# SynthAIr/T-VQ-VAE-TrajGen

Measured on AMD Instinct MI355X. Metric: stage1+stage2 train steps/sec on synthetic (B,C,T) trajectories, 1/2/4/8 GPU, higher is better.
Workload: dtype fp32; 1 GPU; stage1 VQ-VAE + stage2 MaskGIT joint train step, per-GPU batch (B=256,C=6,T=256), K=512, configs/config.yaml architecture; global_batch=256, seq_len=256, parallelism=dp1, launch=hipgraph

## Files before the change

include/tvq.h:

```cpp
#ifndef TVQ_H
#define TVQ_H
#include <stdint.h>

#ifdef __cplusplus
extern "C" {
#endif

#define TVQ_OK 0
#define TVQ_ERR_ARG -1
#define TVQ_ERR_LAUNCH -2

typedef void* tvq_stream_t;

const char* tvq_last_error(void);
int tvq_abi_version(void);
const char* tvq_source_hash(void);
const char* tvq_build_extra(void);
int tvq_counter_pool(int64_t device, int32_t* zeroed, int64_t n);
int tvq_counter_capture(int64_t begin);
int tvq_fill(float* p, int64_t n, float value, tvq_stream_t stream);
int tvq_fill_i64(int64_t* p, int64_t n, int64_t value, tvq_stream_t stream);
int tvq_fill2(float* p, float a, float* q, float b, tvq_stream_t stream);
int tvq_add_i64(int64_t* p, int64_t value, tvq_stream_t stream);
int tvq_sum4(const float* a, const float* b, const float* c, const float* d, float* out,
// ... 307 lines not shown
int tvq_upsample_nearest_bwd(const float* dy, int64_t R, int64_t Lin, int64_t Lout, float* dx,
                             tvq_stream_t stream);
int tvq_gelu_fwd(const float* x, int64_t n, float* y, tvq_stream_t stream);
int tvq_ffn_fwd(const float* xn, const float* r, int64_t M, int64_t D, const float* W1,
                const float* b1, const float* W2, const float* b2, const float* gate, float p,
                const int64_t* seed_ptr, uint64_t offset, float* y, float* pre, float* hd,
                tvq_stream_t stream);
int tvq_ffn_bwd(const float* gy, const float* pre, int64_t M, int64_t D, const float* W1,
                const float* W2, const float* gate, float p, const int64_t* seed_ptr,
                uint64_t offset, float* d_pre, float* dxn, float* gy_gated, tvq_stream_t stream);
int tvq_gelu_bwd(const float* dy, const float* x, int64_t n, float* dx, tvq_stream_t stream);
int64_t tvq_attn_branch_workspace(int64_t B, int64_t D);
int tvq_attn_branch_fwd(const float* x, int64_t B, int64_t S, int64_t D, int64_t heads,
                        const float* g, float nscale, const float* Wqkv, const float* Wo,
                        const float* gate, float drop_p, const int64_t* seed_ptr, uint64_t offset,
                        float* y, float* xn, float* inv, float* qkv, float* o, float* lse,
                        tvq_stream_t stream);
int tvq_attn_branch_bwd(const float* gy, const float* x, int64_t B, int64_t S, int64_t D,
                        int64_t heads, const float* g, float nscale, const float* inv,
                        const float* Wqkv, const float* Wo, const float* gate, float drop_p,
                        const int64_t* seed_ptr, uint64_t offset, const float* qkv, const float* o,
                        const float* lse, float* dx, float* dqkv, float* gy_gated, float* dg,
                        int64_t accumulate, float* workspace, tvq_stream_t stream);


int64_t tvq_prior_lf_eval_workspace(int64_t depth, int64_t K, int64_t n, int64_t n_classes);
int tvq_prior_lf_eval(const int64_t* s, int64_t B, int64_t n, int64_t s_stride,
                      const int64_t* cls_idx, int64_t n_classes, int64_t width,
                      const float* const* weights, int64_t depth, int64_t K, float ln_eps,
                      float* logits, void* workspace, tvq_stream_t stream);
int tvq_prior_lf_eval_sample(const int64_t* s, int64_t B, int64_t n, int64_t s_stride,
                             const int64_t* cls_idx, int64_t n_classes, int64_t width,
                             const float* const* weights, int64_t depth, int64_t K, float ln_eps,
                             int64_t mask_id, const float* gumbel, const int64_t* seed_ptr,
                             uint64_t offset, int64_t* sampled, float* selp, float* logits,
                             void* workspace, int64_t workspace_ready, tvq_stream_t stream);
int tvq_prior_lf_eval_sample_cfg(const int64_t* s, int64_t B, int64_t n, int64_t s_stride,
                                 const int64_t* cls_idx, int64_t n_classes, int64_t width,
                                 const float* const* weights, int64_t depth, int64_t K,
                                 float ln_eps, float cfg_scale, int64_t mask_id,
                                 const float* gumbel, const int64_t* seed_ptr, uint64_t offset,
                                 int64_t* sampled, float* selp, float* logits, void* workspace,
                                 int64_t workspace_ready, tvq_stream_t stream);

int tvq_maskgit_sample(const float* logits, int64_t sb, int64_t sn, int64_t B, int64_t n,
                       int64_t K, const int64_t* s_in, int64_t mask_id, const float* gumbel,
// ... 126 lines not shown
```

t-vq-vae-trajgen_amd/timevqvae/hip/_native.py:

```python
import ctypes
import os
import threading

import torch

_HERE = os.path.dirname(os.path.abspath(__file__))
LIB_PATH = os.environ.get(
    "TVQ_HIP_LIB", os.path.join(os.path.dirname(os.path.dirname(_HERE)), "lib", "libtvq_hip.so"))

P = ctypes.c_void_p
I64 = ctypes.c_int64
I32 = ctypes.c_int
F32 = ctypes.c_float

SIGNATURES = {}
_lib = None
_lock = threading.Lock()


def sig(name, *argtypes, restype=I32):
    SIGNATURES[name] = (list(argtypes), restype)


CSRC = os.path.join(os.path.dirname(os.path.dirname(_HERE)), "csrc")
# ... 142 lines not shown
sig("tvq_attention_fwd", P, I64, P, I64, P, I64, P, I64, P, I64, I64, I64, I64, F32, F32, P, U64, P)
sig("tvq_attention_bwd", P, I64, P, I64, P, I64, P, I64, P, I64, P, I64, I64, I64, I64, F32, F32, P,
    U64, P, P, P, I64, P)
sig("tvq_embedding_fwd", P, I64, I64, P, P, I64, I64, F32, P, U64, P)
sig("tvq_embedding_bwd_workspace", I64, I64, restype=I64)
sig("tvq_embedding_bwd", P, I64, I64, P, I64, I64, P, I64, I64, F32, P, U64, P, P)
sig("tvq_masked_ce_workspace", I64, restype=I64)
sig("tvq_drop_first_token", P, I64, I64, I64, P, I64, P)
sig("tvq_masked_ce_fwd", P, I64, I64, I64, P, P, P, P, P, P)
sig("tvq_masked_ce_bwd", P, I64, I64, I64, P, P, P, P, P, P, I64, P)
sig("tvq_mask_tokens", P, I64, I64, I64, P, U64, P, P, P, P, P)
sig("tvq_upsample_nearest", P, I64, I64, I64, P, P)
sig("tvq_upsample_nearest_bwd", P, I64, I64, I64, P, P)
sig("tvq_gelu_fwd", P, I64, P, P)
sig("tvq_gelu_bwd", P, P, I64, P, P)
sig("tvq_prior_lf_eval_workspace", I64, I64, I64, I64, restype=I64)
sig("tvq_prior_lf_eval", P, I64, I64, I64, P, I64, I64, P, I64, I64, F32, P, P, P)
sig("tvq_ffn_fwd", P, P, I64, I64, P, P, P, P, P, F32, P, U64, P, P, P, P)
sig("tvq_ffn_bwd", P, P, I64, I64, P, P, P, F32, P, U64, P, P, P, P)
sig("tvq_attn_branch_workspace", I64, I64, restype=I64)
sig("tvq_attn_branch_fwd", P, I64, I64, I64, I64, P, F32, P, P, P, F32, P, U64, P, P, P, P, P, P, P)
sig("tvq_attn_branch_bwd", P, P, I64, I64, I64, I64, P, F32, P, P, P, P, F32, P, U64, P, P, P, P, P,
    P, P, I64, P, P)
sig("tvq_prior_lf_eval_sample", P, I64, I64, I64, P, I64, I64, P, I64, I64, F32, I64, P, P, U64,
    P, P, P, P, I64, P)
sig("tvq_prior_lf_eval_sample_cfg", P, I64, I64, I64, P, I64, I64, P, I64, I64, F32, F32, I64, P, P,
    U64, P, P, P, P, I64, P)
sig("tvq_maskgit_sample", P, I64, I64, I64, I64, I64, P, I64, P, P, U64, P, P, P)
sig("tvq_tied_logits_sample_workspace", I64, I64, I64, restype=I64)
sig("tvq_tied_logits_sample", P, I64, I64, P, I64, P, I64, I64, P, I64, P, P, U64, P, P, P, P, P)
sig("tvq_tied_logits_sample_cfg", P, P, I64, I64, P, I64, P, I64, I64, F32, P, I64, P, P, U64, P, P,
    P, P, P)
sig("tvq_maskgit_remask", P, I64, I64, I64, F32, P, P, U64, P, I64, P, P, P)
sig("tvq_conv_packcache_begin", I64, P, I64, P)
sig("tvq_conv_packcache_end")
sig("tvq_conv_packcache_release", I64)
sig("tvq_conv_packcache_pause", I64)
sig("tvq_conv_packcache_entries", restype=I64)
sig("tvq_conv_wgrad_defer_begin")
sig("tvq_conv_wgrad_defer_flush", P)
sig("tvq_wgrad_defer_begin_stream", P)
sig("tvq_conv_wgrad_defer_pause", I64)
sig("tvq_rocket_apply", P, I64, I64, I64, P, P, P, P, P, P, I64, P, P)
sig("tvq_fe_conv1d_out_len", I64, I64, I64, I64, I64, restype=I64)
sig("tvq_fe_ws_weight", P, I64, I64, F32, P, P)
sig("tvq_fe_conv1d", P, I64, I64, I64, P, P, I64, I64, I64, I64, I64, I64, P, P, I64, P)
# ... 123 lines not shown
```

t-vq-vae-trajgen_amd/timevqvae/hip/xf.py:

```python
import contextlib
import math
import os

import torch

from . import rng, streams, wgrad
from ._native import call, grad_sink, ptr, stream_ptr, value
from .conv import _keep
from .linear import _bias_grad_rows, gemm, weight_grad


def _rows(x):
    D = x.shape[-1]
    return x.reshape(-1, D), x.numel() // D, D


class _RMSNorm(torch.autograd.Function):
    @staticmethod
    def forward(ctx, x, g, scale):
        x2, M, D = _rows(x.contiguous())
        y = torch.empty_like(x2)
        inv = torch.empty(M, device=x.device, dtype=torch.float32)
        call("tvq_rmsnorm_fwd", ptr(x2), M, D, ptr(g), float(scale), ptr(y), ptr(inv), stream_ptr())
        ctx.save_for_backward(x2, g, inv)
# ... 272 lines not shown
                        gemm(dqkv, 1, L, xn, D, 1, L, D, M, out=sink, ldc=D, accumulate=True)
            else:
                dW = gemm(dqkv, 1, L, xn, D, 1, L, D, M)
                dws = [dW[i * D:(i + 1) * D] for i in range(3)]
        dwo = weight_grad(gg if gg is not None else g2, o, wo, M, D, D, ctx.wg_tag) if need[5] else None
        return (dx.reshape(B, S, D), None if sink_g is not None else dg, *dws, dwo, None, None, None,
                None)


def attn_branch_supported(x, g, attn):
    if not (FUSED_ATTN and x.is_cuda and x.dim() == 3 and x.shape[-1] == 128 and x.shape[1] <= 32
            and attn.heads == 2):
        return False
    ws = (g, attn.to_q.weight, attn.to_k.weight, attn.to_v.weight, attn.to_out.weight)
    return all(w.dtype == torch.float32 and w.is_cuda and w.is_contiguous() and
               w.data_ptr() % 16 == 0 for w in ws) and tuple(attn.to_q.weight.shape) == (128, 128)


def attn_branch(x, g, attn, gate, p):
    return _AttnBranch.apply(x, g, attn.to_q.weight, attn.to_k.weight, attn.to_v.weight,
                             attn.to_out.weight, gate, int(attn.heads), float(p), int(attn._site))


class _Attention(torch.autograd.Function):
    @staticmethod
    def forward(ctx, q, k, v, heads, drop_p, site):
        B, S, HD = q.shape
        Dh = HD // heads
        q, k, v = q.contiguous(), k.contiguous(), v.contiguous()
        o = torch.empty_like(q)
        lse = torch.empty(B * heads * S, device=q.device)
        seed = rng.seed_tensor(q.device) if drop_p > 0 else None
        off = rng.call_offset(site) if drop_p > 0 else 0
        scale = Dh ** -0.5
        call("tvq_attention_fwd", ptr(q), HD, ptr(k), HD, ptr(v), HD, ptr(o), HD, ptr(lse), B,
             heads, S, Dh, float(scale), float(drop_p), ptr(seed), off, stream_ptr())
        ctx.save_for_backward(q, k, v, o, lse)
        ctx.cfg = (heads, drop_p, off, scale)
        ctx.seed = seed
        return o

    @staticmethod
    def backward(ctx, go):
        q, k, v, o, lse = ctx.saved_tensors
        heads, drop_p, off, scale = ctx.cfg
        B, S, HD = q.shape
# ... 395 lines not shown
```

t-vq-vae-trajgen_amd/timevqvae/models/bidirectional_transformer.py:

```python
import os
import random
from typing import Union

import torch
import torch.nn as nn

from ..hip import rng, streams
from ..hip.conv import PackCache, bn_eval_fusable, conv2d, conv2d_bn_eval
from ..hip.linear import gemm, linear, weight_product
from ..hip.norm import bn_snake
from ..hip.xf import (attn_branch, attn_branch_supported, batch_colsum, drop_first_token,
                      embed_assemble, embedding, fused_ff, fused_ff_supported, gelu,
                      layer_norm, linear_act, masked_cross_entropy, prior_lf_eval,
                      prior_lf_eval_sample,
                      prior_lf_eval_supported, prior_lf_eval_workspace, qkv_attention, rmsnorm, rmsnorm_res,
                      upsample_nearest_t)
from ..hip._native import call, grad_sink, ptr, stream_ptr, value
from ..hip.sample import (codebook_gather_nchw, full_tokens, maskgit_sample, tied_logits_sample,
                          tied_logits_sample_cfg)
from ..hip.upscale import supported as ups_supported
from ..hip.upscale import (hf_embed_folded, hf_embed_supported, upsample_conv_gelu,
                           upsample_conv_gelu_bn_eval)

FUSED_SAMPLE = True
UPS_ON_TOKENS = True
HEAD_FOLD = True
HF_EMBED_FOLD = True


class RMSNorm(nn.Module):
    def __init__(self, dim):
        super().__init__()
        self.scale = dim ** 0.5
        self.g = nn.Parameter(torch.ones(dim))

    def forward(self, x):
        return rmsnorm(x, self.g)
# ... 74 lines not shown
        self.register_buffer("_touched", torch.ones(n), persistent=False)
        for i, layer in enumerate(self.layers):
            for p in layer.parameters():
                p._tvq_gate = (self, i)
        self._site = rng.new_site()
        self._epoch = -1
        self._touched_host = [1.0] * n

    def _draw_branches(self, device):
        from ..hip.optim import grad_epoch
        fresh = self._epoch != grad_epoch()
        self._epoch = grad_epoch()
        n = len(self.layers)
        if rng.decisions_on_device():
            call("tvq_layer_drop", ptr(rng.seed_tensor(device)), rng.call_offset(self._site),
                 float(self.layer_dropout), n, ptr(self._keep), ptr(self._touched),
                 int(not fresh), stream_ptr())
            return None
        keep = [0.0 if random.random() < self.layer_dropout else 1.0 for _ in range(n)]
        self._touched_host = keep if fresh else [max(a, b) for a, b in zip(self._touched_host, keep)]
        self._touched.copy_(torch.tensor(self._touched_host))
        return keep

    def forward(self, x):
        keep = None
        device_gates = False
        if self.training and self.layer_dropout > 0.0:
            keep = self._draw_branches(x.device)
            device_gates = keep is None
        elif self.training and self._touched_host != [1.0] * len(self.layers):
            self._touched_host = [1.0] * len(self.layers)
            self._touched.fill_(1.0)
        for i, (norms, block, _) in enumerate(self.layers):
            if keep is not None and keep[i] == 0.0:
                continue
            gate = self._keep[i:i + 1] if device_gates else None
            if isinstance(norms[0], RMSNorm):
                if isinstance(block, Attention) and attn_branch_supported(x, norms[0].g, block):
                    x = attn_branch(x, norms[0].g, block, gate,
                                    block.dropout if self.training else 0.0)
                    continue
                n, r = rmsnorm_res(x, norms[0].g)
                x = block(n, residual=r, gate=gate)
            else:
                x = block(norms[0](x), residual=x, gate=gate)
        return self.final_norm(x)


class ContinuousTransformerWrapper(nn.Module):
    def __init__(self, dim_in, dim_out, max_seq_len, attn_layers, use_abs_pos_emb=False,
                 post_emb_norm=True):
        super().__init__()
        if use_abs_pos_emb:
            raise NotImplementedError("abs pos emb is off on the path (use_abs_pos_emb=False)")
        dim = attn_layers.dim
        self.max_seq_len = max_seq_len
        self.post_emb_norm = LayerNorm(dim) if post_emb_norm else nn.Identity()
        self.attn_layers = attn_layers
        self.project_in = nn.Linear(dim_in, dim, bias=False)
        self.project_out = nn.Linear(dim, dim_out, bias=False)

    def forward(self, x):
        return self.forward_projected(linear(x, self.project_in.weight))

    def forward_projected(self, x, project_out=True):
        x = self.post_emb_norm(x)
        if not project_out:
            return self.attn_layers(x)
        x = self.attn_layers(x)
        return linear(x, self.project_out.weight)


class _Dropout(torch.autograd.Function):
    @staticmethod
    def forward(ctx, x, p, site):
        x = x.contiguous()
        y = torch.empty_like(x)
        seed = rng.seed_tensor(x.device)
        off = rng.call_offset(site)
        call("tvq_dropout_bwd", ptr(x), x.numel(), float(p), ptr(seed), off, ptr(y), stream_ptr())
        ctx.cfg = (p, off)
        ctx.seed = seed
        return y

    @staticmethod
    def backward(ctx, g):
        p, off = ctx.cfg
        g = g.contiguous()
        dx = torch.empty_like(g)
        call("tvq_dropout_bwd", ptr(g), g.numel(), float(p), ptr(ctx.seed), off, ptr(dx), stream_ptr())
        return dx, None, None

# ... 374 lines not shown
```

Baseline: 260.6 steps/s.

## Fuse D=32 transformer layer (LN, attention, FFN, norms) into one HIP kernel

Adds a whole-layer fused forward and backward kernel for the D=32, single-head, S<=128 transformer blocks. One workgroup per batch element computes the optional post-embedding LayerNorm, RMSNorm, QKV projection, softmax attention with dropout, output projection, residual, the FFN with GELU and dropout, and the optional final norm. Weights stay in registers and K/V in LDS, using MFMA 32x32x2 f32. This removes many small kernel launches and round trips of activations through global memory. The cost is a large, shape-specialised kernel with extra saved tensors, while the weight gradients still go through separate GEMMs.

New measurement: 261.3 steps/s, median of 6. No clear change (+0.3%).

```diff
diff --git a/include/tvq.h b/include/tvq.h
--- a/include/tvq.h
+++ b/include/tvq.h
@@ -353,6 +353,15 @@
                         const int64_t* seed_ptr, uint64_t offset, const float* qkv, const float* o,
                         const float* lse, float* dx, float* dqkv, float* gy_gated, float* dg,
                         int64_t accumulate, float* workspace, tvq_stream_t stream);
+int64_t tvq_xlayer32_workspace(int64_t B);
+int tvq_xlayer32_fwd(const float* x, int64_t B, int64_t S, int64_t D, int64_t heads,
+                     const void* const* params, float p_attn, float p_ff, const int64_t* seed_ptr,
+                     uint64_t off_attn, uint64_t off_ff, void* const* bufs, tvq_stream_t stream);
+int tvq_xlayer32_bwd(const float* gy, const float* x, int64_t B, int64_t S, int64_t D,
+                     int64_t heads, const void* const* params, float p_attn, float p_ff,
+                     const int64_t* seed_ptr, uint64_t off_attn, uint64_t off_ff,
+                     const void* const* saved, void* const* outs, void* const* dgains,
+                     int64_t accumulate_mask, float* workspace, tvq_stream_t stream);
 
 
 int64_t tvq_prior_lf_eval_workspace(int64_t depth, int64_t K, int64_t n, int64_t n_classes);
diff --git a/t-vq-vae-trajgen_amd/csrc/tvq_xlayer32.hip b/t-vq-vae-trajgen_amd/csrc/tvq_xlayer32.hip
--- /dev/null
+++ b/t-vq-vae-trajgen_amd/csrc/tvq_xlayer32.hip
@@ -0,0 +1,709 @@
+#include <math.h>
+
+#include "tvq_common.h"
+#include "tvq_conv_internal.h"
+#include "tvq_ff.h"
+#include "tvq_reduce.h"
+
+namespace tvq {
+
+namespace x32 {
+
+constexpr int D = 32, DH = 64, T = 256, SMAX = 128, LP = 65;
+constexpr int MAT = SMAX * LP;
+constexpr float LN_EPS = 1e-5f;
+
+struct Args {
+  const float *ln_gamma, *g1, *Wq, *Wk, *Wv, *Wo, *gate_a, *g2, *W1, *b1, *W2, *b2, *gate_f, *g3;
+  const float *x, *gy;
+  float *xl, *xn1, *qkv, *o, *lse, *x1, *xn2, *pre, *hd, *x2, *y;
+  float *dx, *dqkv, *gyg_a, *d_pre, *gyg_f, *slab;
+  const int64_t* seed_ptr;
+  uint64_t off_a, off_f;
+  float nscale, scale, p_a, ds_a, p_f, ds_f;
+  int B, S;
+};
+
+__device__ __forceinline__ int wid() { return __builtin_amdgcn_readfirstlane(threadIdx.x >> 6); }
+
+__device__ __forceinline__ bool keep(uint64_t seed, int64_t bh, int S, int i, int j, float p) {
+  return uniform01(seed, ((uint64_t)bh * S + i) * S + j) >= p;
+}
+template <bool KEYS>
+__device__ __forceinline__ uint32_t keep_bits(uint64_t seed, int64_t bh, int S, int q, int k0, int h,
+                                              float p) {
+  uint32_t m = 0;
+#pragma unroll
+  for (int r = 0; r < 16; ++r) {
+    const int o = k0 + ff_crow(r, h);
+    m |= (uint32_t)(KEYS ? keep(seed, bh, S, q, o, p) : keep(seed, bh, S, o, q, p)) << r;
+  }
+  return m;
+}
+__device__ __forceinline__ float gelu(float x) {
+  return 0.5f * x * (1.0f + erff(x * 0.70710678118654752440f));
+}
+__device__ __forceinline__ float gelu_grad(float x) {
+  const float cdf = 0.5f * (1.0f + erff(x * 0.70710678118654752440f));
+  const float pdf = 0.39894228040143267794f * expf(-0.5f * x * x);
+  return cdf + x * pdf;
+}
+
+__device__ __forceinline__ floatx16 load_fm(const float* __restrict__ p, int h) {
+  floatx16 t;
+#pragma unroll
+  for (int g = 0; g < 4; ++g) {
+    const float4 v = *reinterpret_cast<const float4*>(p + 8 * g + 4 * h);
+    t[4 * g] = v.x; t[4 * g + 1] = v.y; t[4 * g + 2] = v.z; t[4 * g + 3] = v.w;
+  }
+  return t;
+}
+__device__ __forceinline__ void store_fm(float* __restrict__ p, int h, const floatx16& t) {
+#pragma unroll
+  for (int g = 0; g < 4; ++g)
+    *reinterpret_cast<float4*>(p + 8 * g + 4 * h) =
+        make_float4(t[4 * g], t[4 * g + 1], t[4 * g + 2], t[4 * g + 3]);
+}
+__device__ __forceinline__ floatx16 wload(const float* __restrict__ W, int ld, int r0, int k0, int lane) {
+  return load_fm(W + (int64_t)(r0 + (lane & 31)) * ld + k0, lane >> 5);
+}
+__device__ __forceinline__ floatx16 wload_t(const float* __restrict__ W, int ld, int k0, int c0, int lane) {
+  floatx16 a;
+  const float* wc = W + c0 + (lane & 31);
+#pragma unroll
+  for (int t = 0; t < 16; ++t) a[t] = wc[(int64_t)(k0 + ff_crow(t, lane >> 5)) * ld];
+  return a;
+}
+__device__ __forceinline__ floatx16 mma16(const floatx16& a, const floatx16& b, floatx16 acc) {
+#pragma unroll
+  for (int t = 0; t < 16; ++t) acc = __builtin_amdgcn_mfma_f32_32x32x2f32(a[t], b[t], acc, 0, 0, 0);
+  return acc;
+}
+__device__ __forceinline__ floatx16 mma_rows(const float* __restrict__ M, int r0, int c0, int lane,
+                                             const floatx16& b, floatx16 acc) {
+  const float* m = M + (r0 + (lane & 31)) * LP + c0 + 4 * (lane >> 5);
+#pragma unroll
+  for (int t = 0; t < 16; ++t)
+    acc = __builtin_amdgcn_mfma_f32_32x32x2f32(m[(t & 3) + 8 * (t >> 2)], b[t], acc, 0, 0, 0);
+  return acc;
+}
+__device__ __forceinline__ bool live(int S, int r0, int g) { return r0 + 8 * g < S; }
+__device__ __forceinline__ floatx16 mma_cols(const float* __restrict__ M, int r0, int c0, int lane,
+                                             const floatx16& b, floatx16 acc, int S) {
+  const float* m = M + (r0 + 4 * (lane >> 5)) * LP + c0 + (lane & 31);
+#pragma unroll
+  for (int g = 0; g < 4; ++g)
+    if (live(S, r0, g))
+#pragma unroll
+      for (int e = 0; e < 4; ++e)
+        acc = __builtin_amdgcn_mfma_f32_32x32x2f32(m[(e + 8 * g) * LP], b[4 * g + e], acc, 0, 0, 0);
+  return acc;
+}
+__device__ __forceinline__ void stage(float* __restrict__ M, int tok, int c0, int h, const floatx16& t) {
+#pragma unroll
+  for (int r = 0; r < 16; ++r) M[tok * LP + c0 + ff_crow(r, h)] = t[r];
+}
+__device__ __forceinline__ float half_sum(float v) { return v + __shfl_xor(v, 32, 64); }
+
+__device__ __forceinline__ float rms_inv(const floatx16& x) {
+  float ss = 0.f;
+#pragma unroll
+  for (int r = 0; r < 16; ++r) ss += x[r] * x[r];
+  return 1.0f / fmaxf(sqrtf(half_sum(ss)), 1e-12f);
+}
+__device__ __forceinline__ floatx16 rms_fwd(const floatx16& x, const floatx16& g, float inv, float nscale) {
+  floatx16 y;
+#pragma unroll
+  for (int r = 0; r < 16; ++r) y[r] = x[r] * inv * nscale * g[r];
+  return y;
+}
+__device__ __forceinline__ floatx16 rms_bwd(const floatx16& dn, const floatx16& x, const floatx16& g,
+                                            float nscale, bool valid, floatx16& dg) {
+  const float inv = rms_inv(x);
+  float dp = 0.f;
+#pragma unroll
+  for (int r = 0; r < 16; ++r) dp += dn[r] * g[r] * x[r];
+  dp = half_sum(dp);
+  const float c = dp * nscale * inv * inv * inv;
+  floatx16 dx;
+#pragma unroll
+  for (int r = 0; r < 16; ++r) {
+    dx[r] = dn[r] * g[r] * nscale * inv - x[r] * c;
+    dg[r] = valid ? dn[r] * x[r] * inv * nscale : 0.f;
+  }
+  return dx;
+}
+__device__ __forceinline__ floatx16 ln_hat(const floatx16& x, float& rstd) {
+  float s = 0.f;
+#pragma unroll
+  for (int r = 0; r < 16; ++r) s += x[r];
+  const float mean = half_sum(s) / (float)D;
+  floatx16 t;
+  float q = 0.f;
+#pragma unroll
+  for (int r = 0; r < 16; ++r) {
+    t[r] = x[r] - mean;
+    q = fmaf(t[r], t[r], q);
+  }
+  rstd = 1.0f / sqrtf(half_sum(q) / (float)D + LN_EPS);
+#pragma unroll
+  for (int r = 0; r < 16; ++r) t[r] *= rstd;
+  return t;
+}
+
+constexpr int F_TOT = 2 * MAT;
+
+template <bool DROP>
+__global__ __launch_bounds__(T) void xlayer32_fwd_kernel(Args a) {
+  extern __shared__ float sm[];
+  float* Kl = sm;
+  float* Vl = sm + MAT;
+  const int lane = threadIdx.x & 63, j = lane & 31, h = lane >> 5, w = wid();
+  const int b = blockIdx.x, S = a.S, nt = (S + 31) >> 5;
+  const int tok = 32 * w + j;
+  const bool valid = tok < S, active = w < nt;
+  const int64_t row = (int64_t)b * S + (valid ? tok : S - 1);
+  floatx16 xl, qt[2];
+  floatx16 wo[2], w1, w2, g2, b1, b2, g3;
+  if (active) {
+    xl = load_fm(a.x + row * D, h);
+    floatx16 wq[2], wk[2], wv[2];
+#pragma unroll
+    for (int c = 0; c < 2; ++c) {
+      wq[c] = wload(a.Wq, D, 32 * c, 0, lane);
+      wk[c] = wload(a.Wk, D, 32 * c, 0, lane);
+      wv[c] = wload(a.Wv, D, 32 * c, 0, lane);
+    }
+    const floatx16 g1 = load_fm(a.g1, h);
+    const floatx16 gm = load_fm(a.ln_gamma ? a.ln_gamma : a.g1, h);
+    __builtin_amdgcn_sched_barrier(0);
+    if (a.ln_gamma) {
+      float rstd;
+      const floatx16 xh = ln_hat(xl, rstd);
+#pragma unroll
+      for (int r = 0; r < 16; ++r) xl[r] = xh[r] * gm[r];
+      if (valid) store_fm(a.xl + row * D, h, xl);
+    }
+    const floatx16 xn = rms_fwd(xl, g1, rms_inv(xl), a.nscale);
+    if (valid) store_fm(a.xn1 + row * D, h, xn);
+    float* qr = a.qkv + row * 3 * DH;
+#pragma unroll
+    for (int c = 0; c < 2; ++c) {
+      qt[c] = mma16(wq[c], xn, ff_zero());
+      const floatx16 kt = mma16(wk[c], xn, ff_zero());
+      const floatx16 vt = mma16(wv[c], xn, ff_zero());
+      if (valid) {
+        store_fm(qr + 32 * c, h, qt[c]);
+        store_fm(qr + DH + 32 * c, h, kt);
+        store_fm(qr + 2 * DH + 32 * c, h, vt);
+      }
+      stage(Kl, tok, 32 * c, h, kt);
+      stage(Vl, tok, 32 * c, h, vt);
+    }
+    wo[0] = wload(a.Wo, DH, 0, 0, lane);
+    wo[1] = wload(a.Wo, DH, 0, 32, lane);
+    w1 = wload(a.W1, D, 0, 0, lane);
+    w2 = wload(a.W2, D, 0, 0, lane);
+    g2 = load_fm(a.g2, h);
+    b1 = load_fm(a.b1, h);
+    b2 = load_fm(a.b2, h);
+    g3 = load_fm(a.g3 ? a.g3 : a.g2, h);
+    __builtin_amdgcn_sched_barrier(0);
+  }
+  __syncthreads();
+  if (!active) return;
+  const uint64_t seed_a = DROP ? mix_seed(a.seed_ptr, a.off_a) : 0ull;
+  floatx16 s[4];
+  uint32_t kb[4];
+#pragma unroll
+  for (int kw = 0; kw < 4; ++kw) {
+    s[kw] = ff_zero();
+    kb[kw] = 0;
+    if (kw < nt) {
+      if (DROP) kb[kw] = keep_bits<true>(seed_a, b, S, tok, 32 * kw, h, a.p_a);
+      s[kw] = mma_rows(Kl, 32 * kw, 0, lane, qt[0], s[kw]);
+      s[kw] = mma_rows(Kl, 32 * kw, 32, lane, qt[1], s[kw]);
+    }
+  }
+  float mx = -INFINITY;
+#pragma unroll
+  for (int kw = 0; kw < 4; ++kw)
+#pragma unroll
+    for (int r = 0; r < 16; ++r) {
+      const int key = 32 * kw + ff_crow(r, h);
+      s[kw][r] = key < S ? s[kw][r] * a.scale : -INFINITY;
+      mx = fmaxf(mx, s[kw][r]);
+    }
+  mx = fmaxf(mx, __shfl_xor(mx, 32, 64));
+  float sum = 0.f;
+#pragma unroll
+  for (int kw = 0; kw < 4; ++kw)
+    if (kw < nt)
+#pragma unroll
+      for (int g = 0; g < 4; ++g)
+#pragma unroll
+        for (int e = 0; e < 4; ++e) {
+          const int r = 4 * g + e;
+          s[kw][r] = live(S, 32 * kw, g) ? expf(s[kw][r] - mx) : 0.f;
+          sum += s[kw][r];
+        }
+  sum = half_sum(sum);
+  const float isum = 1.0f / sum;
+  if (h == 0 && valid) a.lse[(int64_t)b * S + tok] = mx + logf(sum);
+#pragma unroll
+  for (int kw = 0; kw < 4; ++kw)
+    if (kw < nt)
+#pragma unroll
+      for (int r = 0; r < 16; ++r) {
+        float pv = s[kw][r] * isum;
+        if (DROP) pv = (valid & ((kb[kw] >> r) & 1u)) ? pv * a.ds_a : 0.f;
+        s[kw][r] = pv;
+      }
+  floatx16 yt = ff_zero();
+#pragma unroll
+  for (int c = 0; c < 2; ++c) {
+    floatx16 ot = ff_zero();
+#pragma unroll
+    for (int kw = 0; kw < 4; ++kw)
+      if (kw < nt) ot = mma_cols(Vl, 32 * kw, 32 * c, lane, s[kw], ot, S);
+    if (valid) store_fm(a.o + row * DH + 32 * c, h, ot);
+    yt = mma16(wo[c], ot, yt);
+  }
+  floatx16 x1;
+  {
+    const float gt = a.gate_a ? *a.gate_a : 1.0f;
+#pragma unroll
+    for (int r = 0; r < 16; ++r) {
+      float v = yt[r];
+      if (a.gate_a) v *= gt;
+      x1[r] = v + xl[r];
+    }
+  }
+  if (valid) store_fm(a.x1 + row * D, h, x1);
+  const floatx16 xn2 = rms_fwd(x1, g2, rms_inv(x1), a.nscale);
+  if (valid) store_fm(a.xn2 + row * D, h, xn2);
+  floatx16 pre = mma16(w1, xn2, ff_zero());
+  const uint64_t seed_f = a.p_f > 0.f ? mix_seed(a.seed_ptr, a.off_f) : 0ull;
+  floatx16 hd;
+#pragma unroll
+  for (int r = 0; r < 16; ++r) {
+    pre[r] += b1[r];
+    float v = gelu(pre[r]);
+    if (a.p_f > 0.f)
+      v = uniform01(seed_f, (uint64_t)(row * D + ff_crow(r, h))) >= a.p_f ? v * a.ds_f : 0.f;
+    hd[r] = v;
+  }
+  if (valid) {
+    store_fm(a.pre + row * D, h, pre);
+    store_fm(a.hd + row * D, h, hd);
+  }
+  const floatx16 y2 = mma16(w2, hd, ff_zero());
+  floatx16 x2;
+  {
+    const float gt = a.gate_f ? *a.gate_f : 1.0f;
+#pragma unroll
+    for (int r = 0; r < 16; ++r) {
+      float v = y2[r] + b2[r];
+      if (a.gate_f) v *= gt;
+      x2[r] = v + x1[r];
+    }
+  }
+  if (a.g3) {
+    if (valid) store_fm(a.x2 + row * D, h, x2);
+    x2 = rms_fwd(x2, g3, rms_inv(x2), a.nscale);
+  }
+  if (valid) store_fm(a.y + row * D, h, x2);
+}
+
+constexpr int B_DQ = 2 * MAT, B_LS = B_DQ + SMAX, B_RED = B_LS + SMAX, B_TOT = B_RED + 4 * 4 * D;
+
+__device__ __forceinline__ void token_sum(floatx16 v, float* __restrict__ red, int j, int h) {
+#pragma unroll
+  for (int o = 1; o < 32; o <<= 1) {
+    floatx16 t;
+#pragma unroll
+    for (int r = 0; r < 16; ++r) t[r] = __shfl_xor(v[r], o, 64);
+#pragma unroll
+    for (int r = 0; r < 16; ++r) v[r] += t[r];
+  }
+  if (j == 0) {
+#pragma unroll
+    for (int r = 0; r < 16; ++r) red[ff_crow(r, h)] = v[r];
+  }
+}
+
+template <bool DROP>
+__global__ __launch_bounds__(T) void xlayer32_bwd_kernel(Args a) {
+  extern __shared__ float sm[];
+  float* Kl = sm;
+  float* Vl = sm + MAT;
+  float* Ql = sm;
+  float* Gl = sm + MAT;
+  const int lane = threadIdx.x & 63, j = lane & 31, h = lane >> 5, w = wid();
+  const int b = blockIdx.x, S = a.S, nt = (S + 31) >> 5;
+  const int tok = 32 * w + j;
+  const bool valid = tok < S, active = w < nt;
+  const int64_t row = (int64_t)b * S + (valid ? tok : S - 1);
+  floatx16 g, qt[2], kt[2], vt[2], dot[2];
+  float Dq = 0.f;
+  if (active) {
+    g = load_fm(a.gy + row * D, h);
+    const floatx16 x2r = load_fm((a.g3 ? a.x2 : a.x1) + row * D, h);
+    const floatx16 g3 = load_fm(a.g3 ? a.g3 : a.g2, h), g2 = load_fm(a.g2, h);
+    const floatx16 w2t = wload_t(a.W2, D, 0, 0, lane), w1t = wload_t(a.W1, D, 0, 0, lane);
+    const floatx16 pre = load_fm(a.pre + row * D, h), x1r = load_fm(a.x1 + row * D, h);
+    floatx16 wot[2], ot[2];
+    {
+      const float* qr = a.qkv + row * 3 * DH;
+#pragma unroll
+      for (int c = 0; c < 2; ++c) {
+        wot[c] = wload_t(a.Wo, DH, 0, 32 * c, lane);
+        ot[c] = load_fm(a.o + row * DH + 32 * c, h);
+        qt[c] = load_fm(qr + 32 * c, h);
+        kt[c] = load_fm(qr + DH + 32 * c, h);
+        vt[c] = load_fm(qr + 2 * DH + 32 * c, h);
+      }
+    }
+    __builtin_amdgcn_sched_barrier(0);
+    if (a.g3) {
+      floatx16 dg;
+      g = rms_bwd(g, x2r, g3, a.nscale, valid, dg);
+      token_sum(dg, sm + B_RED + (3 * 4 + w) * D, j, h);
+    }
+    floatx16 gg;
+    {
+      const float gt = a.gate_f ? *a.gate_f : 1.0f;
+#pragma unroll
+      for (int r = 0; r < 16; ++r) gg[r] = a.gate_f ? g[r] * gt : g[r];
+    }
+    if (valid) store_fm(a.gyg_f + row * D, h, gg);
+    floatx16 dp = mma16(w2t, gg, ff_zero());
+    {
+      const uint64_t seed_f = a.p_f > 0.f ? mix_seed(a.seed_ptr, a.off_f) : 0ull;
+#pragma unroll
+      for (int r = 0; r < 16; ++r) {
+        float v = dp[r];
+        if (a.p_f > 0.f)
+          v = uniform01(seed_f, (uint64_t)(row * D + ff_crow(r, h))) >= a.p_f ? v * a.ds_f : 0.f;
+        dp[r] = v * gelu_grad(pre[r]);
+      }
+    }
+    if (valid) store_fm(a.d_pre + row * D, h, dp);
+    const floatx16 dn2 = mma16(w1t, dp, ff_zero());
+    {
+      floatx16 dg;
+      const floatx16 d1 = rms_bwd(dn2, x1r, g2, a.nscale, valid, dg);
+      token_sum(dg, sm + B_RED + (2 * 4 + w) * D, j, h);
+#pragma unroll
+      for (int r = 0; r < 16; ++r) g[r] += d1[r];
+    }
+    {
+      const float gt = a.gate_a ? *a.gate_a : 1.0f;
+#pragma unroll
+      for (int r = 0; r < 16; ++r) gg[r] = a.gate_a ? g[r] * gt : g[r];
+    }
+    if (valid) store_fm(a.gyg_a + row * D, h, gg);
+#pragma unroll
+    for (int c = 0; c < 2; ++c) {
+      dot[c] = mma16(wot[c], gg, ff_zero());
+#pragma unroll
+      for (int r = 0; r < 16; ++r) {
+        if (!valid) dot[c][r] = 0.f;
+        Dq = fmaf(dot[c][r], ot[c][r], Dq);
+      }
+      stage(Kl, tok, 32 * c, h, kt[c]);
+      stage(Vl, tok, 32 * c, h, vt[c]);
+    }
+    Dq = half_sum(Dq);
+    if (h == 0) {
+      sm[B_DQ + tok] = Dq;
+      sm[B_LS + tok] = valid ? a.lse[(int64_t)b * S + tok] : 0.f;
+    }
+  }
+  __syncthreads();
+  const uint64_t seed_a = DROP ? mix_seed(a.seed_ptr, a.off_a) : 0ull;
+  floatx16 dq[2];
+  if (active) {
+#pragma unroll
+    for (int c = 0; c < 2; ++c) dq[c] = ff_zero();
+    const float lq = sm[B_LS + tok];
+#pragma unroll
+    for (int kw = 0; kw < 4; ++kw)
+      if (kw < nt) {
+        const uint32_t kb = DROP ? keep_bits<true>(seed_a, b, S, tok, 32 * kw, h, a.p_a) : 0u;
+        floatx16 sc = mma_rows(Kl, 32 * kw, 0, lane, qt[0], ff_zero());
+        sc = mma_rows(Kl, 32 * kw, 32, lane, qt[1], sc);
+        floatx16 dp = mma_rows(Vl, 32 * kw, 0, lane, dot[0], ff_zero());
+        dp = mma_rows(Vl, 32 * kw, 32, lane, dot[1], dp);
+        floatx16 ds = ff_zero();
+#pragma unroll
+        for (int g = 0; g < 4; ++g)
+          if (live(S, 32 * kw, g))
+#pragma unroll
+            for (int e = 0; e < 4; ++e) {
+              const int r = 4 * g + e, key = 32 * kw + ff_crow(r, h);
+              const float p = expf(sc[r] * a.scale - lq);
+              float d = dp[r];
+              if (DROP) d = ((kb >> r) & 1u) ? d * a.ds_a : 0.f;
+              ds[r] = ((key < S) & valid) ? p * (d - Dq) : 0.f;
+            }
+        dq[0] = mma_cols(Kl, 32 * kw, 0, lane, ds, dq[0], S);
+        dq[1] = mma_cols(Kl, 32 * kw, 32, lane, ds, dq[1], S);
+      }
+  }
+  __syncthreads();
+  if (active) {
+#pragma unroll
+    for (int c = 0; c < 2; ++c) {
+      stage(Ql, tok, 32 * c, h, qt[c]);
+      stage(Gl, tok, 32 * c, h, dot[c]);
+    }
+  }
+  __syncthreads();
+  if (active) {
+    floatx16 dk[2], dv[2];
+#pragma unroll
+    for (int c = 0; c < 2; ++c) dk[c] = dv[c] = ff_zero();
+#pragma unroll
+    for (int qw = 0; qw < 4; ++qw)
+      if (qw < nt) {
+        const uint32_t kb = DROP ? keep_bits<false>(seed_a, b, S, tok, 32 * qw, h, a.p_a) : 0u;
+        floatx16 sc = mma_rows(Ql, 32 * qw, 0, lane, kt[0], ff_zero());
+        sc = mma_rows(Ql, 32 * qw, 32, lane, kt[1], sc);
+        floatx16 dp = mma_rows(Gl, 32 * qw, 0, lane, vt[0], ff_zero());
+        dp = mma_rows(Gl, 32 * qw, 32, lane, vt[1], dp);
+        floatx16 ds = ff_zero(), pd = ff_zero();
+#pragma unroll
+        for (int g = 0; g < 4; ++g)
+          if (live(S, 32 * qw, g))
+#pragma unroll
+            for (int e = 0; e < 4; ++e) {
+              const int r = 4 * g + e, ql = 32 * qw + ff_crow(r, h);
+              const bool on = (ql < S) & valid;
+              const float p = expf(sc[r] * a.scale - sm[B_LS + ql]);
+              float d = dp[r], pq = p;
+              if (DROP) {
+                const bool kp = (kb >> r) & 1u;
+                pq = kp ? p * a.ds_a : 0.f;
+                d = kp ? d * a.ds_a : 0.f;
+              }
+              ds[r] = on ? p * (d - sm[B_DQ + ql]) : 0.f;
+              pd[r] = on ? pq : 0.f;
+            }
+#pragma unroll
+        for (int c = 0; c < 2; ++c) {
+          dk[c] = mma_cols(Ql, 32 * qw, 32 * c, lane, ds, dk[c], S);
+          dv[c] = mma_cols(Gl, 32 * qw, 32 * c, lane, pd, dv[c], S);
+        }
+      }
+    floatx16 wqt[2], wkt[2], wvt[2];
+#pragma unroll
+    for (int c = 0; c < 2; ++c) {
+      wqt[c] = wload_t(a.Wq, D, 32 * c, 0, lane);
+      wkt[c] = wload_t(a.Wk, D, 32 * c, 0, lane);
+      wvt[c] = wload_t(a.Wv, D, 32 * c, 0, lane);
+    }
+    const floatx16 xlr = load_fm((a.ln_gamma ? a.xl : a.x) + row * D, h), g1 = load_fm(a.g1, h);
+    const floatx16 xr = load_fm(a.x + row * D, h), gm = load_fm(a.ln_gamma ? a.ln_gamma : a.g1, h);
+    __builtin_amdgcn_sched_barrier(0);
+    floatx16 dn1 = ff_zero();
+    float* dr = a.dqkv + row * 3 * DH;
+#pragma unroll
+    for (int c = 0; c < 2; ++c) {
+#pragma unroll
+      for (int r = 0; r < 16; ++r) {
+        dq[c][r] *= a.scale;
+        dk[c][r] *= a.scale;
+      }
+      if (valid) {
+        store_fm(dr + 32 * c, h, dq[c]);
+        store_fm(dr + DH + 32 * c, h, dk[c]);
+        store_fm(dr + 2 * DH + 32 * c, h, dv[c]);
+      }
+      dn1 = mma16(wqt[c], dq[c], dn1);
+      dn1 = mma16(wkt[c], dk[c], dn1);
+      dn1 = mma16(wvt[c], dv[c], dn1);
+    }
+    {
+      floatx16 dg;
+      const floatx16 d0 = rms_bwd(dn1, xlr, g1, a.nscale, valid, dg);
+      token_sum(dg, sm + B_RED + (1 * 4 + w) * D, j, h);
+#pragma unroll
+      for (int r = 0; r < 16; ++r) g[r] += d0[r];
+    }
+    if (a.ln_gamma) {
+      float rstd;
+      const floatx16 xh = ln_hat(xr, rstd);
+      floatx16 dg;
+      float s1 = 0.f, s2 = 0.f;
+#pragma unroll
+      for (int r = 0; r < 16; ++r) {
+        dg[r] = valid ? g[r] * xh[r] : 0.f;
+        g[r] *= gm[r];
+        s1 += g[r];
+        s2 += g[r] * xh[r];
+      }
+      s1 = half_sum(s1) / (float)D;
+      s2 = half_sum(s2) / (float)D;
+#pragma unroll
+      for (int r = 0; r < 16; ++r) g[r] = rstd * (g[r] - s1 - xh[r] * s2);
+      token_sum(dg, sm + B_RED + (0 * 4 + w) * D, j, h);
+    }
+    if (valid) store_fm(a.dx + row * D, h, g);
+  }
+  __syncthreads();
+  if (threadIdx.x < 4 * D) {
+    const int k = threadIdx.x >> 5, f = threadIdx.x & 31;
+    const bool on = k == 0 ? a.ln_gamma != nullptr : k == 3 ? a.g3 != nullptr : true;
+    if (on) {
+      float t = 0.f;
+      for (int q = 0; q < nt; ++q) t += sm[B_RED + (k * 4 + q) * D + f];
+      a.slab[((int64_t)k * a.B + b) * D + f] = t;
+    }
+  }
+}
+
+static bool aligned(const void* p) { return ((uintptr_t)p & 15) == 0; }
+
+static bool params_ok(const void* const* P) {
+  for (int i = 0; i < 14; ++i) {
+    const bool opt = i == 0 || i == 6 || i == 12 || i == 13;
+    if (!P[i] && !opt) return false;
+    if (i != 6 && i != 12 && !aligned(P[i])) return false;
+  }
+  return true;
+}
+
+static void set_params(Args& a, const void* const* P) {
+  const float* const* p = reinterpret_cast<const float* const*>(P);
+  a.ln_gamma = p[0]; a.g1 = p[1]; a.Wq = p[2]; a.Wk = p[3]; a.Wv = p[4]; a.Wo = p[5];
+  a.gate_a = p[6]; a.g2 = p[7]; a.W1 = p[8]; a.b1 = p[9]; a.W2 = p[10]; a.b2 = p[11];
+  a.gate_f = p[12]; a.g3 = p[13];
+}
+
+static void set_dropout(Args& a, float p_attn, float p_ff, const int64_t* seed_ptr, uint64_t off_a,
+                        uint64_t off_f) {
+  a.seed_ptr = seed_ptr; a.off_a = off_a; a.off_f = off_f;
+  a.p_a = p_attn; a.ds_a = p_attn > 0.f ? 1.0f / (1.0f - p_attn) : 1.0f;
+  a.p_f = p_ff; a.ds_f = p_ff > 0.f ? 1.0f / (1.0f - p_ff) : 1.0f;
+  a.nscale = sqrtf((float)D); a.scale = 0.125f;
+}
+
+}
+}
+
+using namespace tvq;
+
+extern "C" int64_t tvq_xlayer32_workspace(int64_t B) {
+  return 4 * (B * x32::D + reduce_rows_scratch(B, x32::D));
+}
+
+extern "C" int tvq_xlayer32_fwd(const float* x, int64_t B, int64_t S, int64_t D, int64_t heads,
+                                const void* const* params, float p_attn, float p_ff,
+                                const int64_t* seed_ptr, uint64_t off_attn, uint64_t off_ff,
+                                void* const* bufs, tvq_stream_t stream) {
+  using namespace x32;
+  TVQ_CHECK_ARG(x && params && bufs && B > 0, "tvq_xlayer32_fwd: bad arguments");
+  TVQ_CHECK_ARG(D == x32::D && heads == 1 && S >= 1 && S <= SMAX,
+                "tvq_xlayer32_fwd: needs D = 32, 1 head of 64, S <= 128");
+  TVQ_CHECK_ARG(p_attn >= 0.f && p_attn < 1.f && p_ff >= 0.f && p_ff < 1.f &&
+                    ((p_attn == 0.f && p_ff == 0.f) || seed_ptr),
+                "tvq_xlayer32_fwd: bad dropout");
+  TVQ_CHECK_ARG(params_ok(params) && aligned(x),
+                "tvq_xlayer32_fwd: parameters must be present and 16-byte aligned");
+  Args a = {};
+  set_params(a, params);
+  float* const* o = reinterpret_cast<float* const*>(bufs);
+  for (int i = 0; i < 11; ++i) {
+    const bool opt = (i == 0 && !a.ln_gamma) || (i == 9 && !a.g3);
+    TVQ_CHECK_ARG((o[i] || opt) && aligned(o[i]),
+                  "tvq_xlayer32_fwd: outputs must be present and 16-byte aligned");
+  }
+  a.x = x;
+  a.xl = o[0]; a.xn1 = o[1]; a.qkv = o[2]; a.o = o[3]; a.lse = o[4]; a.x1 = o[5]; a.xn2 = o[6];
+  a.pre = o[7]; a.hd = o[8]; a.x2 = o[9]; a.y = o[10];
+  set_dropout(a, p_attn, p_ff, seed_ptr, off_attn, off_ff);
+  a.B = (int)B; a.S = (int)S;
+  static bool attr = [] {
+    (void)hipFuncSetAttribute((const void*)xlayer32_fwd_kernel<false>,
+                              hipFuncAttributeMaxDynamicSharedMemorySize, F_TOT * 4);
+    (void)hipFuncSetAttribute((const void*)xlayer32_fwd_kernel<true>,
+                              hipFuncAttributeMaxDynamicSharedMemorySize, F_TOT * 4);
+    return true;
+  }();
+  (void)attr;
+  if (p_attn > 0.f)
+    hipLaunchKernelGGL(xlayer32_fwd_kernel<true>, dim3((unsigned)B), dim3(T), F_TOT * 4,
+                       (hipStream_t)stream, a);
+  else
+    hipLaunchKernelGGL(xlayer32_fwd_kernel<false>, dim3((unsigned)B), dim3(T), F_TOT * 4,
+                       (hipStream_t)stream, a);
+  TVQ_PLAN("xlayer32_fwd B%lld S%lld ln%d fin%d", (long long)B, (long long)S, a.ln_gamma != nullptr,
+           a.g3 != nullptr);
+  return launch_status("tvq_xlayer32_fwd");
+}
+
+extern "C" int tvq_xlayer32_bwd(const float* gy, const float* x, int64_t B, int64_t S, int64_t D,
+                                int64_t heads, const void* const* params, float p_attn, float p_ff,
+                                const int64_t* seed_ptr, uint64_t off_attn, uint64_t off_ff,
+                                const void* const* saved, void* const* outs, void* const* dgains,
+                                int64_t accumulate_mask, float* workspace, tvq_stream_t stream) {
+  using namespace x32;
+  TVQ_CHECK_ARG(gy && x && params && saved && outs && dgains && workspace && B > 0,
+                "tvq_xlayer32_bwd: bad arguments");
+  TVQ_CHECK_ARG(D == x32::D && heads == 1 && S >= 1 && S <= SMAX,
+                "tvq_xlayer32_bwd: needs D = 32, 1 head of 64, S <= 128");
+  TVQ_CHECK_ARG(p_attn >= 0.f && p_attn < 1.f && p_ff >= 0.f && p_ff < 1.f &&
+                    ((p_attn == 0.f && p_ff == 0.f) || seed_ptr),
+                "tvq_xlayer32_bwd: bad dropout");
+  TVQ_CHECK_ARG(params_ok(params) && aligned(gy) && aligned(x) && aligned(workspace),
+                "tvq_xlayer32_bwd: parameters must be present and 16-byte aligned");
+  Args a = {};
+  set_params(a, params);
+  float* const* sv = reinterpret_cast<float* const*>(const_cast<void* const*>(saved));
+  for (int i = 0; i < 7; ++i) {
+    const bool opt = (i == 0 && !a.ln_gamma) || (i == 6 && !a.g3);
+    TVQ_CHECK_ARG((sv[i] || opt) && aligned(sv[i]),
+                  "tvq_xlayer32_bwd: saved tensors must be present and 16-byte aligned");
+  }
+  float* const* o = reinterpret_cast<float* const*>(outs);
+  for (int i = 0; i < 5; ++i)
+    TVQ_CHECK_ARG(o[i] && aligned(o[i]),
+                  "tvq_xlayer32_bwd: outputs must be present and 16-byte aligned");
+  a.gy = gy; a.x = x;
+  a.xl = sv[0]; a.qkv = sv[1]; a.o = sv[2]; a.lse = sv[3]; a.x1 = sv[4]; a.pre = sv[5]; a.x2 = sv[6];
+  a.dx = o[0]; a.dqkv = o[1]; a.gyg_a = o[2]; a.d_pre = o[3]; a.gyg_f = o[4];
+  a.slab = workspace;
+  set_dropout(a, p_attn, p_ff, seed_ptr, off_attn, off_ff);
+  a.B = (int)B; a.S = (int)S;
+  hipStream_t st = (hipStream_t)stream;
+  static bool attr = [] {
+    (void)hipFuncSetAttribute((const void*)xlayer32_bwd_kernel<false>,
+                              hipFuncAttributeMaxDynamicSharedMemorySize, B_TOT * 4);
+    (void)hipFuncSetAttribute((const void*)xlayer32_bwd_kernel<true>,
+                              hipFuncAttributeMaxDynamicSharedMemorySize, B_TOT * 4);
+    return true;
+  }();
+  (void)attr;
+  if (p_attn > 0.f)
+    hipLaunchKernelGGL(xlayer32_bwd_kernel<true>, dim3((unsigned)B), dim3(T), B_TOT * 4, st, a);
+  else
+    hipLaunchKernelGGL(xlayer32_bwd_kernel<false>, dim3((unsigned)B), dim3(T), B_TOT * 4, st, a);
+  TVQ_PLAN("xlayer32_bwd B%lld S%lld ln%d fin%d", (long long)B, (long long)S, a.ln_gamma != nullptr,
+           a.g3 != nullptr);
+  int rc = launch_status("tvq_xlayer32_bwd");
+  if (rc) return rc;
+  float* const* dg = reinterpret_cast<float* const*>(dgains);
+  const float* const gains[4] = {a.ln_gamma, a.g1, a.g2, a.g3};
+  float* scratch = workspace + 4 * B * x32::D;
+  const int64_t rs = reduce_rows_scratch(B, x32::D);
+  for (int k = 0; k < 4; ++k) {
+    if (!dg[k] || !gains[k]) continue;
+    const float* slab = workspace + k * B * x32::D;
+    if ((accumulate_mask >> k) & 1)
+      param_rows_finish(slab, B, x32::D, dg[k], 1, scratch + k * rs, st);
+    else
+      reduce_rows(slab, B, x32::D, x32::D, dg[k], nullptr, 0, 0, scratch + k * rs, st);
+  }
+  return launch_status("tvq_xlayer32_bwd");
+}
diff --git a/t-vq-vae-trajgen_amd/timevqvae/hip/_native.py b/t-vq-vae-trajgen_amd/timevqvae/hip/_native.py
--- a/t-vq-vae-trajgen_amd/timevqvae/hip/_native.py
+++ b/t-vq-vae-trajgen_amd/timevqvae/hip/_native.py
@@ -188,6 +188,9 @@
 sig("tvq_attn_branch_fwd", P, I64, I64, I64, I64, P, F32, P, P, P, F32, P, U64, P, P, P, P, P, P, P)
 sig("tvq_attn_branch_bwd", P, P, I64, I64, I64, I64, P, F32, P, P, P, P, F32, P, U64, P, P, P, P, P,
     P, P, I64, P, P)
+sig("tvq_xlayer32_workspace", I64, restype=I64)
+sig("tvq_xlayer32_fwd", P, I64, I64, I64, I64, P, F32, F32, P, U64, U64, P, P)
+sig("tvq_xlayer32_bwd", P, P, I64, I64, I64, I64, P, F32, F32, P, U64, U64, P, P, P, I64, P, P)
 sig("tvq_prior_lf_eval_sample", P, I64, I64, I64, P, I64, I64, P, I64, I64, F32, I64, P, P, U64,
     P, P, P, P, I64, P)
 sig("tvq_prior_lf_eval_sample_cfg", P, I64, I64, I64, P, I64, I64, P, I64, I64, F32, F32, I64, P, P,
diff --git a/t-vq-vae-trajgen_amd/timevqvae/hip/xf.py b/t-vq-vae-trajgen_amd/timevqvae/hip/xf.py
--- a/t-vq-vae-trajgen_amd/timevqvae/hip/xf.py
+++ b/t-vq-vae-trajgen_amd/timevqvae/hip/xf.py
@@ -318,6 +318,139 @@
                              attn.to_out.weight, gate, int(attn.heads), float(p), int(attn._site))
 
 
+FUSED_LAYER32 = True
+
+
+def _ptr_array(ts):
+    import ctypes
+    return (ctypes.c_void_p * len(ts))(*[ptr(t) for t in ts])
+
+
+class _Layer32(torch.autograd.Function):
+
+    @staticmethod
+    def forward(ctx, x, ln_gamma, g1, wq, wk, wv, wo, gate_a, g2, w1, b1, w2, b2, gate_f, g3,
+                p_attn, site_a, p_ff, site_f):
+        B, S, D = x.shape
+        M = B * S
+        dev = x.device
+        x2 = x.reshape(M, D).contiguous()
+        rows = torch.empty((M * (7 * D + 64 + 192 + 1),), device=dev)
+        cuts, at = [], 0
+        for width in (D, D, D, D, D, D, D, 64, 192):
+            cuts.append(rows[at:at + M * width].view(M, width))
+            at += M * width
+        xl, xn1, x1, xn2, pre, hd, xe, o, qkv = cuts
+        lse = rows[at:at + M]
+        y = torch.empty((M, D), device=dev)
+        if ln_gamma is None:
+            xl = None
+        if g3 is None:
+            xe = None
+        seed = rng.seed_tensor(dev) if (p_attn > 0 or p_ff > 0) else None
+        off_a = rng.call_offset(site_a) if p_attn > 0 else 0
+        off_f = rng.call_offset(site_f) if p_ff > 0 else 0
+        params = (ln_gamma, g1, wq, wk, wv, wo, gate_a, g2, w1, b1, w2, b2, gate_f, g3)
+        call("tvq_xlayer32_fwd", ptr(x2), B, S, D, 1, _ptr_array(params), float(p_attn),
+             float(p_ff), ptr(seed), off_a, off_f,
+             _ptr_array((xl, xn1, qkv, o, lse, x1, xn2, pre, hd, xe, y)), stream_ptr())
+        ctx.save_for_backward(x2, xl, xn1, qkv, o, lse, x1, xn2, pre, hd, xe)
+        ctx.params = params
+        ctx.seed = seed
+        ctx.cfg = (B, S, D, float(p_attn), float(p_ff), off_a, off_f)
+        ctx.wg_tag = wgrad.current_tag()
+        return y.view(B, S, D)
+
+    @staticmethod
+    def backward(ctx, gy):
+        x2, xl, xn1, qkv, o, lse, x1, xn2, pre, hd, xe = ctx.saved_tensors
+        B, S, D, p_attn, p_ff, off_a, off_f = ctx.cfg
+        ln_gamma, g1, wq, wk, wv, wo, gate_a, g2, w1, b1, w2, b2, gate_f, g3 = ctx.params
+        M, L = B * S, 192
+        dev = x2.device
+        need = ctx.needs_input_grad
+        g2d = gy.reshape(M, D).contiguous()
+        dx = torch.empty((M, D), device=dev)
+        outs = torch.empty((M * (3 * D + L),), device=dev)
+        gga, d_pre, ggf = (outs[i * M * D:(i + 1) * M * D].view(M, D) for i in range(3))
+        dqkv = outs[3 * M * D:].view(M, L)
+        gains = [(ln_gamma, need[1]), (g1, need[2]), (g2, need[8]), (g3, need[14])]
+        dgs, ret, mask = [], [], 0
+        for k, (g, want) in enumerate(gains):
+            if g is None or not want:
+                dgs.append(None)
+                ret.append(None)
+                continue
+            sink = grad_sink(g)
+            dgs.append(sink if sink is not None else torch.empty(D, device=dev))
+            ret.append(None if sink is not None else dgs[-1])
+            mask |= int(sink is not None) << k
+        ws = torch.empty(value("tvq_xlayer32_workspace", B), device=dev)
+        call("tvq_xlayer32_bwd", ptr(g2d), ptr(x2), B, S, D, 1, _ptr_array(ctx.params), p_attn,
+             p_ff, ptr(ctx.seed), off_a, off_f, _ptr_array((xl, qkv, o, lse, x1, pre, xe)),
+             _ptr_array((dx, dqkv, gga, d_pre, ggf)), _ptr_array(dgs), mask, ptr(ws), stream_ptr())
+        _keep(ws)
+        dws = [None, None, None]
+        if any(need[3:6]):
+            sinks = [grad_sink(w) if n else None for w, n in zip((wq, wk, wv), need[3:6])]
+            sink = _stacked(sinks, (L, D)) if all(s_ is not None for s_ in sinks) else None
+            if sink is not None:
+                if not wgrad.defer(dqkv, L, xn1, D, sink, D, L, D, M, ctx.wg_tag):
+                    with streams.offload(dqkv, xn1):
+                        gemm(dqkv, 1, L, xn1, D, 1, L, D, M, out=sink, ldc=D, accumulate=True)
+            else:
+                for i, (w, n) in enumerate(zip((wq, wk, wv), need[3:6])):
+                    if n:
+                        dws[i] = weight_grad(dqkv[:, 64 * i:64 * (i + 1)].contiguous(), xn1, w, M,
+                                             64, D, ctx.wg_tag)
+        dwo = weight_grad(gga, o, wo, M, D, 64, ctx.wg_tag) if need[6] else None
+
+        def lin(g, xin, w, b, nw, nb):
+            if nw and nb:
+                return weight_grad(g, xin, w, M, D, D, ctx.wg_tag, b)
+            return (weight_grad(g, xin, w, M, D, D, ctx.wg_tag) if nw else None,
+                    _bias_grad_rows(g, grad_sink(b)) if nb else None)
+
+        dw1, db1 = lin(d_pre, xn2, w1, b1, need[9], need[10])
+        dw2, db2 = lin(ggf, hd, w2, b2, need[11], need[12])
+        return (dx.view(B, S, D) if need[0] else None, ret[0], ret[1], *dws, dwo, None, ret[2],
+                dw1, db1, dw2, db2, None, ret[3], None, None, None, None)
+
+
+def layer32_supported(x, attn, ff, norms, ln=None, final=None):
+    if not (FUSED_LAYER32 and x.is_cuda and x.dim() == 3 and x.shape[-1] == 32
+            and 1 <= x.shape[1] <= 128 and x.dtype == torch.float32):
+        return False
+    if x.is_contiguous() and x.data_ptr() % 16 != 0:
+        return False
+    if not (hasattr(attn, "to_q") and attn.heads == 1 and tuple(attn.to_q.weight.shape) == (64, 32)
+            and tuple(attn.to_out.weight.shape) == (32, 64) and hasattr(ff, "ff")):
+        return False
+    lin1, lin2 = ff.ff[0][0], ff.ff[2]
+    if not (tuple(lin1.weight.shape) == (32, 32) and tuple(lin2.weight.shape) == (32, 32)
+            and lin1.bias is not None and lin2.bias is not None):
+        return False
+    gains = [n for n in (*norms, final) if n is not None]
+    if not all(hasattr(n, "g") and hasattr(n, "scale") for n in gains):
+        return False
+    if ln is not None and not hasattr(ln, "gamma"):
+        return False
+    ws = [n.g for n in gains] + [attn.to_q.weight, attn.to_k.weight, attn.to_v.weight,
+                                 attn.to_out.weight, lin1.weight, lin1.bias, lin2.weight, lin2.bias]
+    if ln is not None:
+        ws.append(ln.gamma)
+    return all(_param16(w) for w in ws)
+
+
+def layer32(x, attn, ff, norms, gate_a, gate_f, ln=None, final=None):
+    lin1, lin2 = ff.ff[0][0], ff.ff[2]
+    return _Layer32.apply(x, None if ln is None else ln.gamma, norms[0].g, attn.to_q.weight,
+                          attn.to_k.weight, attn.to_v.weight, attn.to_out.weight, gate_a,
+                          norms[1].g, lin1.weight, lin1.bias, lin2.weight, lin2.bias, gate_f,
+                          None if final is None else final.g, float(attn.dropout),
+                          int(attn._site), float(ff.ff[1].p), int(ff._site))
+
+
 class _Attention(torch.autograd.Function):
     @staticmethod
     def forward(ctx, q, k, v, heads, drop_p, site):
diff --git a/t-vq-vae-trajgen_amd/timevqvae/models/bidirectional_transformer.py b/t-vq-vae-trajgen_amd/timevqvae/models/bidirectional_transformer.py
--- a/t-vq-vae-trajgen_amd/timevqvae/models/bidirectional_transformer.py
+++ b/t-vq-vae-trajgen_amd/timevqvae/models/bidirectional_transformer.py
@@ -11,8 +11,8 @@
 from ..hip.norm import bn_snake
 from ..hip.xf import (attn_branch, attn_branch_supported, batch_colsum, drop_first_token,
                       embed_assemble, embedding, fused_ff, fused_ff_supported, gelu,
-                      layer_norm, linear_act, masked_cross_entropy, prior_lf_eval,
-                      prior_lf_eval_sample,
+                      layer32, layer32_supported, layer_norm, linear_act, masked_cross_entropy,
+                      prior_lf_eval, prior_lf_eval_sample,
                       prior_lf_eval_supported, prior_lf_eval_workspace, qkv_attention, rmsnorm, rmsnorm_res,
                       upsample_nearest_t)
 from ..hip._native import call, grad_sink, ptr, stream_ptr, value
@@ -133,7 +133,7 @@
         self._touched.copy_(torch.tensor(self._touched_host))
         return keep
 
-    def forward(self, x):
+    def forward(self, x, pre=None):
         keep = None
         device_gates = False
         if self.training and self.layer_dropout > 0.0:
@@ -142,10 +142,29 @@
         elif self.training and self._touched_host != [1.0] * len(self.layers):
             self._touched_host = [1.0] * len(self.layers)
             self._touched.fill_(1.0)
+        n_layers = len(self.layers)
+        skip = -1
         for i, (norms, block, _) in enumerate(self.layers):
+            if i == skip:
+                continue
+            gate = self._keep[i:i + 1] if device_gates else None
+            if (self.training and isinstance(block, Attention) and i + 1 < n_layers
+                    and (keep is None or (keep[i] != 0.0 and keep[i + 1] != 0.0))):
+                nf, ff, _ = self.layers[i + 1]
+                ln = pre if isinstance(pre, LayerNorm) else None
+                final = self.final_norm if i + 2 == n_layers else None
+                if (pre is None or ln is not None) and layer32_supported(
+                        x, block, ff, (norms[0], nf[0]), ln, final):
+                    x = layer32(x, block, ff, (norms[0], nf[0]), gate,
+                                self._keep[i + 1:i + 2] if device_gates else None, ln, final)
+                    pre, skip = None, i + 1
+                    if final is not None:
+                        return x
+                    continue
+            if pre is not None:
+                x, pre = pre(x), None
             if keep is not None and keep[i] == 0.0:
                 continue
-            gate = self._keep[i:i + 1] if device_gates else None
             if isinstance(norms[0], RMSNorm):
                 if isinstance(block, Attention) and attn_branch_supported(x, norms[0].g, block):
                     x = attn_branch(x, norms[0].g, block, gate,
@@ -155,6 +174,8 @@
                 x = block(n, residual=r, gate=gate)
             else:
                 x = block(norms[0](x), residual=x, gate=gate)
+        if pre is not None:
+            x = pre(x)
         return self.final_norm(x)
 
 
@@ -175,10 +196,9 @@
         return self.forward_projected(linear(x, self.project_in.weight))
 
     def forward_projected(self, x, project_out=True):
-        x = self.post_emb_norm(x)
+        x = self.attn_layers(x, pre=self.post_emb_norm)
         if not project_out:
-            return self.attn_layers(x)
-        x = self.attn_layers(x)
+            return x
         return linear(x, self.project_out.weight)
 
 
```
